# vsislab/Controllable_XGating

Measured on AMD Instinct MI355X. Metric: decoder timesteps/sec (train fwd+bwd) at batch 128, MSRVTT 26x1536+1024, higher is better.
Workload: dtype f32; 1 GPU; configs[1]: 1xMI355X batch 128 per GPU teacher-forced XE train, 26 frames x (1536+1024), hidden 512, att 1536, emb 468, vocab 20000, seq_len 20 (T=21), fp32; global_batch=128, per_gpu_batch=128, parallelism=dp1, gemm_precision=fp32, zero_grad=fused into the update, launch=eager kernel launches

## Files before the change

controllable_xgating_amd/csrc/xg_heads.hip:

```cpp
#include "xg_common.h"
#include "xg_kernels.h"
#include "xg_select.h"
#include <type_traits>
#include <cstdlib>

namespace {

constexpr int RT = 1024;

__device__ __forceinline__ float block_max(float v, float* red) {
    v = wave_max(v);
    const int lane = threadIdx.x & 63, wave = threadIdx.x >> 6;
    __syncthreads();
    if (lane == 0) red[wave] = v;
    __syncthreads();
    float r = red[0];
    for (int i = 1; i < (int)(blockDim.x >> 6); ++i) r = fmaxf(r, red[i]);
    return r;
}
__device__ __forceinline__ float block_sum(float v, float* red) {
    v = wave_sum(v);
    const int lane = threadIdx.x & 63, wave = threadIdx.x >> 6;
    __syncthreads();
    if (lane == 0) red[wave] = v;
// ... 110 lines not shown
    const float m = mask[i] * (mask2 ? mask2[i] : 1.f);
    dlogp[(size_t)i * V + tgt_of(target, b, t, T, roll)] = -scale * (scale_dev ? scale_dev[0] : 1.f) * m / sums[1];
}

__device__ __forceinline__ float reward_mask(const int64_t* seq, int ld_seq, int b, int t, int n) {
    if (t >= n) return 0.f;
    return (t == 0 || seq[(size_t)b * ld_seq + t - 1] > 0) ? 1.f : 0.f;
}
__global__ void reward_fwd_kernel(const float* slp, int ld_slp, const int64_t* seq, int ld_seq, const float* reward, int rs_b,
                                  int rs_t, const int32_t* n_dev, int m, int L, float* out2) {
    __shared__ float red[256 / 64];
    const int i = blockIdx.x * 256 + threadIdx.x;
    const int n = n_dev ? min(max(*n_dev, 0), L) : L;
    float a = 0.f, k = 0.f;
    if (i < m * L) {
        const int b = i / L, t = i % L;
        k = reward_mask(seq, ld_seq, b, t, n);
        if (k != 0.f) a = -slp[(size_t)b * ld_slp + t] * reward[(size_t)b * rs_b + (size_t)t * rs_t];
    }
    a = block_sum(a, red);
    k = block_sum(k, red);
    if (threadIdx.x == 0) { atomicAdd(out2, a); atomicAdd(out2 + 1, k); }
}
__global__ void reward_bwd_kernel(const int64_t* seq, int ld_seq, const float* reward, int rs_b, int rs_t, const int32_t* n_dev,
                                  int m, int L, const float* sums, const float* scale_dev, float* dslp, int ld_d) {
    const int i = blockIdx.x * 256 + threadIdx.x;
    if (i >= m * L) return;
    const int n = n_dev ? min(max(*n_dev, 0), L) : L;
    const int b = i / L, t = i % L;
    const float k = reward_mask(seq, ld_seq, b, t, n);
    dslp[(size_t)b * ld_d + t] = k != 0.f ? -(scale_dev ? scale_dev[0] : 1.f) * reward[(size_t)b * rs_b + (size_t)t * rs_t] / sums[1] : 0.f;
}

__device__ __forceinline__ void xent_row_finish(float mx, float s, float* red, const float* x, int i, int b, int t, int T,
                                                const int64_t* seq, const float* mask, const float* mask2, int roll,
                                                float* lse_out, float* sums2) {
    const float gmx = block_max(mx, red);
    s = (mx == -INFINITY) ? 0.f : s * expf(mx - gmx);
    s = block_sum(s, red);
    if (threadIdx.x == 0) {
        const float lse = gmx + logf(s);
        lse_out[i] = lse;
        const float m = mask[(size_t)b * T + t] * (mask2 ? mask2[(size_t)b * T + t] : 1.f);
        const int64_t tg = tgt_of(seq, b, t, T, roll);
        atomicAdd(sums2, -(x[tg] - lse) * m);
        atomicAdd(sums2 + 1, m);
    }
}
__global__ void __launch_bounds__(RT) xent_fwd_kernel(const float* __restrict__ logits, int ld, const int64_t* seq,
                                                        const float* mask, const float* mask2, int B, int T, int V,
                                                        int roll, float* lse_out, float* sums2, int row0) {
    __shared__ float red[RT / 64];
    const int i = row0 + blockIdx.x, t = i / B, b = i % B;
    const float* x = logits + (size_t)i * ld;
    float mx = -INFINITY, s = 0.f;
    for (int v0 = threadIdx.x; v0 < V; v0 += 8 * RT) {
        float xv[8];
#pragma unroll
        for (int j = 0; j < 8; ++j) { const int v = v0 + j * RT; xv[j] = v < V ? x[v] : -INFINITY; }
        float bm = xv[0];
#pragma unroll
        for (int j = 1; j < 8; ++j) bm = fmaxf(bm, xv[j]);
        if (bm > mx) { s *= expf(mx - bm); mx = bm; }
        if (mx > -INFINITY) {
#pragma unroll
            for (int j = 0; j < 8; ++j) s += expf(xv[j] - mx);
        }
    }
    xent_row_finish(mx, s, red, x, i, b, t, T, seq, mask, mask2, roll, lse_out, sums2);
}
template <int NV4>
__global__ void __launch_bounds__(RT) xent_fwd_reg_kernel(const float* __restrict__ logits, int ld, const int64_t* seq,
                                                            const float* mask, const float* mask2, int B, int T, int V,
                                                            int roll, float* lse_out, float* sums2, int row0) {
    __shared__ float red[RT / 64];
    const int i = row0 + blockIdx.x, t = i / B, b = i % B;
    const float* x = logits + (size_t)i * ld;
    float4 xv[NV4];
#pragma unroll
    for (int j = 0; j < NV4; ++j) {
        const int v = (threadIdx.x + j * RT) * 4;
        if (v + 3 < V) xv[j] = *reinterpret_cast<const float4*>(x + v);
        else {
            xv[j].x = v < V ? x[v] : -INFINITY;         xv[j].y = v + 1 < V ? x[v + 1] : -INFINITY;
            xv[j].z = v + 2 < V ? x[v + 2] : -INFINITY; xv[j].w = -INFINITY;
        }
    }
    float mx = -INFINITY;
#pragma unroll
    for (int j = 0; j < NV4; ++j) mx = fmaxf(fmaxf(mx, fmaxf(xv[j].x, xv[j].y)), fmaxf(xv[j].z, xv[j].w));
    float s = 0.f;
    if (mx > -INFINITY) {
#pragma unroll
        for (int j = 0; j < NV4; ++j) s += (expf(xv[j].x - mx) + expf(xv[j].y - mx)) + (expf(xv[j].z - mx) + expf(xv[j].w - mx));
    }
    xent_row_finish(mx, s, red, x, i, b, t, T, seq, mask, mask2, roll, lse_out, sums2);
}
template <bool BF>
__global__ void __launch_bounds__(RT) xent_bwd_kernel(float* __restrict__ logits, int ld, const int64_t* seq,
                                                        const float* mask, const float* mask2, int B, int T, int V,
                                                        int roll, const float* lse, const float* sums2,
                                                        const float* scale_dev, float scale, int row0, unsigned short* d16) {
    const int i = row0 + blockIdx.x, t = i / B, b = i % B;
    float* x = logits + (size_t)i * ld;
    const float m = mask[(size_t)b * T + t] * (mask2 ? mask2[(size_t)b * T + t] : 1.f);
    const float coef = (scale_dev ? scale_dev[0] : 1.f) * scale * m / sums2[1];
    const int64_t tg = tgt_of(seq, b, t, T, roll);
    const float l = lse[i];
    for (int v = threadIdx.x; v < V; v += RT) {
        const float pv = expf(x[v] - l);
        const float gv = coef * (pv - (v == tg ? 1.f : 0.f));
        x[v] = gv;
        if (BF) {
            unsigned u = __float_as_uint(gv);
            u += 0x7FFFu + ((u >> 16) & 1u);
            d16[(size_t)i * ld + v] = (unsigned short)(u >> 16);
        }
    }
}

template <int NV4, bool BF>
__global__ void __launch_bounds__(RT) xent_bwd_reg_kernel(float* __restrict__ logits, int ld, const int64_t* seq,
                                                            const float* mask, const float* mask2, int B, int T, int V,
                                                            int roll, const float* lse, const float* sums2,
                                                            const float* scale_dev, float scale, int row0, unsigned short* d16) {
    const int i = row0 + blockIdx.x, t = i / B, b = i % B;
    float* x = logits + (size_t)i * ld;
    float4 xv[NV4];
#pragma unroll
// ... 731 lines not shown
    else if (npt <= 16) hipLaunchKernelGGL((log_softmax_reg_kernel<16>), dim3(rows), dim3(RT), 0, st, in, ldin, out, ldout, V, inner, outer, pm);
    else if (npt <= 24) hipLaunchKernelGGL((log_softmax_reg_kernel<24>), dim3(rows), dim3(RT), 0, st, in, ldin, out, ldout, V, inner, outer, pm);
    else hipLaunchKernelGGL(log_softmax_kernel, dim3(rows), dim3(RT), 0, st, in, ldin, out, ldout, V, inner, outer, pm);
    XG_CHECK_LAUNCH();
    return XG_OK;
}
int xgk_log_softmax_bwd(hipStream_t st, const float* dlogp, const float* logp, int ldp, float* dlogits, int ldd,
                        int rows, int V, int inner, int outer, int permute) {
    if (rows <= 0) return XG_OK;
    const int npt = xg_cdiv(V, RT);
    if (npt <= 8) hipLaunchKernelGGL((log_softmax_bwd_reg_kernel<8>), dim3(rows), dim3(RT), 0, st, dlogp, logp, ldp, dlogits, ldd, V, inner, outer, permute);
    else if (npt <= 16) hipLaunchKernelGGL((log_softmax_bwd_reg_kernel<16>), dim3(rows), dim3(RT), 0, st, dlogp, logp, ldp, dlogits, ldd, V, inner, outer, permute);
    else if (npt <= 24) hipLaunchKernelGGL((log_softmax_bwd_reg_kernel<24>), dim3(rows), dim3(RT), 0, st, dlogp, logp, ldp, dlogits, ldd, V, inner, outer, permute);
    else hipLaunchKernelGGL(log_softmax_bwd_kernel, dim3(rows), dim3(RT), 0, st, dlogp, logp, ldp, dlogits, ldd, V, inner, outer, permute);
    XG_CHECK_LAUNCH();
    return XG_OK;
}
int xgk_nll_fwd(hipStream_t st, const float* logp, const int64_t* target, const float* mask, const float* mask2,
                int B, int T, int V, int roll, float* out2) {
    if (hipMemsetAsync(out2, 0, 2 * sizeof(float), st) != hipSuccess) return XG_EHIP;
    hipLaunchKernelGGL(nll_fwd_kernel, dim3(xg_cdiv(B * T, 256)), dim3(256), 0, st, logp, target, mask, mask2, B, T, V,
                       roll, out2);
    XG_CHECK_LAUNCH();
    return XG_OK;
}
int xgk_nll_bwd(hipStream_t st, const int64_t* target, const float* mask, const float* mask2, int B, int T, int V,
                int roll, const float* sums, float scale, const float* scale_dev, float* dlogp) {
    if (hipMemsetAsync(dlogp, 0, sizeof(float) * (size_t)B * T * V, st) != hipSuccess) return XG_EHIP;
    hipLaunchKernelGGL(nll_bwd_kernel, dim3(xg_cdiv(B * T, 256)), dim3(256), 0, st, target, mask, mask2, B, T, V, roll,
                       sums, scale, scale_dev, dlogp);
    XG_CHECK_LAUNCH();
    return XG_OK;
}
int xgk_xent_fwd(hipStream_t st, const float* logits, int ld, const int64_t* seq, const float* mask,
                 const float* mask2, int B, int T, int V, int roll, float* lse, float* sums2, int row0, int nrows,
                 bool zero_sums) {
    if (zero_sums && hipMemsetAsync(sums2, 0, 2 * sizeof(float), st) != hipSuccess) return XG_EHIP;
    if (nrows < 0) nrows = B * T - row0;
    if (nrows <= 0) return XG_OK;
    const bool al = ((uintptr_t)logits % 16 == 0) && ld % 4 == 0;
#define XG_XENT_REG(NV4_) hipLaunchKernelGGL((xent_fwd_reg_kernel<NV4_>), dim3(nrows), dim3(RT), 0, st, logits, ld, seq, mask, mask2, B, T, V, roll, lse, sums2, row0)
    if (al && V <= 2 * 4096) XG_XENT_REG(2);
    else if (al && V <= 5 * 4096) XG_XENT_REG(5);
    else if (al && V <= 8 * 4096) XG_XENT_REG(8);
    else hipLaunchKernelGGL(xent_fwd_kernel, dim3(nrows), dim3(RT), 0, st, logits, ld, seq, mask, mask2, B, T, V, roll, lse, sums2, row0);
#undef XG_XENT_REG
    XG_CHECK_LAUNCH();
    return XG_OK;
}
int xgk_xent_bwd(hipStream_t st, float* logits_inout, int ld, const int64_t* seq, const float* mask,
                 const float* mask2, int B, int T, int V, int roll, const float* lse, const float* sums2,
                 const float* scale_dev, float scale, int row0, int nrows, unsigned short* d16) {
    if (nrows < 0) nrows = B * T - row0;
    if (nrows <= 0) return XG_OK;
    const bool al = ((uintptr_t)logits_inout % 16 == 0) && ld % 4 == 0 && (!d16 || (uintptr_t)d16 % 8 == 0);
#define XG_XENT_BREG(NV4_) do { \
        if (d16) hipLaunchKernelGGL((xent_bwd_reg_kernel<NV4_, true>), dim3(nrows), dim3(RT), 0, st, logits_inout, ld, seq, mask, mask2, B, T, V, \
                                    roll, lse, sums2, scale_dev, scale, row0, d16); \
        else hipLaunchKernelGGL((xent_bwd_reg_kernel<NV4_, false>), dim3(nrows), dim3(RT), 0, st, logits_inout, ld, seq, mask, mask2, B, T, V, \
                                roll, lse, sums2, scale_dev, scale, row0, d16); } while (0)
    if (al && V > 1024 && V <= 2 * 4096) XG_XENT_BREG(2);
    else if (al && V > 1024 && V <= 5 * 4096) XG_XENT_BREG(5);
    else if (al && V > 1024 && V <= 8 * 4096) XG_XENT_BREG(8);
    else if (d16) hipLaunchKernelGGL(xent_bwd_kernel<true>, dim3(nrows), dim3(RT), 0, st, logits_inout, ld, seq, mask, mask2, B, T, V, roll,
                                     lse, sums2, scale_dev, scale, row0, d16);
    else hipLaunchKernelGGL(xent_bwd_kernel<false>, dim3(nrows), dim3(RT), 0, st, logits_inout, ld, seq, mask, mask2, B, T, V, roll,
                            lse, sums2, scale_dev, scale, row0, d16);
#undef XG_XENT_BREG
    XG_CHECK_LAUNCH();
    return XG_OK;
}
int xgk_choose(hipStream_t st, const float* logp, int B, int V, int mode, const float* uniforms,
               const int64_t* forced, int64_t forced_stride, float temperature, int64_t* tok, float* tok_logp) {
    hipLaunchKernelGGL(choose_kernel, dim3(B), dim3(RT), 0, st, logp, V, mode, uniforms, forced, forced_stride,
                       temperature, tok, tok_logp);
    XG_CHECK_LAUNCH();
    return XG_OK;
}
int xgk_rollout_step(hipStream_t st, int B, const float* logits, const float* uniforms, const int64_t* forced,
// ... 119 lines not shown
```

controllable_xgating_amd/csrc/xg_kernels.h:

```cpp
#pragma once
#include "xg_common.h"
#include "xg_select.h"
#include <cstddef>

static inline int xgk_group_rows(int k_depth) {
    const int g = 4096 / (k_depth > 0 ? k_depth : 1);
    return g < 1 ? 1 : (g > 8 ? 8 : g);
}
enum { XGK_GEMM_BG = 0x100,
       XGK_GEMM_ALONE = 0x200 };
int xgk_gemm(hipStream_t st, int mode, bool transA, bool transB, int M, int N, int K, const float* A, int lda,
             const float* B, int ldb, float* C, int ldc, const float* bias, bool relu, bool accumulate);
int xgk_gemm_cs(hipStream_t st, int mode, bool transA, bool transB, int M, int N, int K, const float* A, int lda,
                const float* B, int ldb, float* C, int ldc, const float* bias, bool relu, bool accumulate, float* cs1, float* cs2,
                float* cs3);
int xgk_gemm_x(hipStream_t st, int mode, bool transA, bool transB, int M, int N, int K, const float* A, const unsigned short* A16,
               int lda, const float* B, const unsigned short* B16, int ldb, float* C, int ldc, const float* bias, bool relu,
               bool accumulate, float* cs1 = nullptr, float* cs2 = nullptr, float* cs3 = nullptr);
int xgk_gemm_bf16(hipStream_t st, int planes, bool transA, bool transB, int M, int N, int K, const float* A, int lda,
                  const float* B, int ldb, float* C, int ldc, const float* bias, bool relu, bool accumulate, float* cs1 = nullptr,
                  float* cs2 = nullptr, float* cs3 = nullptr);
int xgk_gemm_bf16x(hipStream_t st, int planes, bool transA, bool transB, int M, int N, int K, const float* A, const unsigned short* A16,
                   int lda, const float* B, const unsigned short* B16, int ldb, float* C, int ldc, const float* bias, bool relu,
                   bool accumulate, float* cs1 = nullptr, float* cs2 = nullptr, float* cs3 = nullptr);
// ... 164 lines not shown
int xgk_dstep_err_word();
bool xgk_dstep_ok(const XgDims& d);
int xgk_dstep(hipStream_t st, DStepArgs& a, int gemm_mode);

enum { PK_H2A1 = 0, PK_H2A2, PK_DGATE, PK_L1_I2H, PK_L1_A2H, PK_L1_H2H, PK_L2_I2H, PK_L2_A2H, PK_L2_H2H, PK_ENC_RGB, PK_ENC_OPFL,
       PKB_L2_A2H, PKB_L2_H2H, PKB_H2A2, PKB_L1_H2H, PKB_ENC_RGB, PKB_ENC_OPFL, PKB_L2_I2H, PKB_H2A1, PK_COUNT };
enum { W16_LOGIT = 0, W16_EMB_RGB, W16_EMB_OPFL, W16_WIH_RGB, W16_WIH_OPFL, W16_GATE_RGB, W16_GATE_OPFL, W16_FUSION, W16_V2A,
       W16_DGATE, W16_L1_I2H, W16_L1_A2H, W16_COUNT };
struct PackedView { const float* m[PK_COUNT]; int nck[PK_COUNT]; int dtype;
                    const unsigned short* w16[W16_COUNT]; };
size_t xgk_packed_floats(const XgDims& d);
size_t xgk_packed_total_bytes(const XgDims& d, int dtype);
bool xgk_packed_view(const XgDims& d, const void* packed, int dtype, PackedView* v);

int xgk_attn_fwd(hipStream_t st, const float* p, const float* vproj, const float* V, const float* w, float* alpha,
                 float* af, int B, int K, int R, int A, bool half_cu = false);
int xgk_attn_bwd(hipStream_t st, const float* daf, int lddaf, const float* p, const float* vproj, const float* V,
                 const float* w, const float* alpha, float* de, float* dp, int B, int K, int R, int A);
int xgk_attn_bwd_post(hipStream_t st, const float* P , const float* vproj, const float* w,
                      const float* DE , float* dvproj, float* dw, int T, int B, int K, int A);
int xgk_attn_post_dV(hipStream_t st, const float* P, const float* vproj, const float* w, const float* DE, float* dvproj, float* dw,
                     const float* ALPHA, const float* DAF, int lddaf, int64_t daf_tstride, float* dV, int T, int B, int K, int A, int R);
int xgk_attn_dV(hipStream_t st, const float* ALPHA , const float* DAF , int lddaf,
                int64_t daf_tstride, float* dV, int T, int B, int K, int R, bool accumulate);

int xgk_log_softmax(hipStream_t st, const float* in, int ldin, float* out, int ldout, int rows, int V, int inner,
                    int outer, bool permute);
int xgk_log_softmax_bwd(hipStream_t st, const float* dlogp, const float* logp, int ldp, float* dlogits, int ldd,
                        int rows, int V, int inner, int outer, int permute);
int xgk_nll_fwd(hipStream_t st, const float* logp, const int64_t* target, const float* mask, const float* mask2,
                int B, int T, int V, int roll, float* out2);
int xgk_nll_bwd(hipStream_t st, const int64_t* target, const float* mask, const float* mask2, int B, int T, int V,
                int roll, const float* sums, float scale, const float* scale_dev, float* dlogp);
int xgk_xent_fwd(hipStream_t st, const float* logits, int ld, const int64_t* seq, const float* mask,
                 const float* mask2, int B, int T, int V, int roll, float* lse, float* sums2, int row0 = 0,
                 int nrows = -1, bool zero_sums = true);
int xgk_xent_bwd(hipStream_t st, float* logits_inout, int ld, const int64_t* seq, const float* mask,
                 const float* mask2, int B, int T, int V, int roll, const float* lse, const float* sums2,
                 const float* scale_dev, float scale, int row0 = 0, int nrows = -1, unsigned short* d16 = nullptr);
int xgk_choose(hipStream_t st, const float* logp, int B, int V, int mode, const float* uniforms,
               const int64_t* forced, int64_t forced_stride, float temperature, int64_t* tok, float* tok_logp);
int xgk_rollout_step(hipStream_t st, int B, const float* logits, const float* uniforms, const int64_t* forced,
                     int64_t fstride, const float* unf_prev, const float* table, int64_t* tok, float* tok_logp, float* unf,
                     float* lse, int64_t* seq, float* seq_logp, int32_t* maxf, float* xt, float temperature, int V, int E,
                     int t, int T, int mode, int split);
int xgk_rollout_finalize(hipStream_t st, const int32_t* maxf, int32_t* n_steps, int Tm1, int nparts);
bool xgk_vocab_select_ok(int B, int R, int V, const float* H, int ldh, const float* W);
int xgk_vocab_tile_width(int V);
int xgk_vocab_part(hipStream_t st, int B, int R, int V, const float* H, int ldh, const float* W, const float* bias, float* logits,
                   int wr_rows, float* part, float temperature);
RollSelectArgs xgk_roll_select_args(const float* logits, const float* part, const float* uniforms, const int64_t* forced, int64_t fstride,
                                    const float* unf_prev, const float* table, int64_t* tok, float* tok_logp, float* unf, float* lse,
                                    int64_t* seq, float* seq_logp, int32_t* maxf, float* xt, float temperature, int V, int E, int t, int T,
                                    int mode, int split);
int xgk_roll_select(hipStream_t st, int B, const float* logits, const float* part, const float* uniforms, const int64_t* forced,
                    int64_t fstride, const float* unf_prev, const float* table, int64_t* tok, float* tok_logp, float* unf,
                    float* lse, int64_t* seq, float* seq_logp, int32_t* maxf, float* xt, float temperature, int V, int E,
                    int t, int T, int mode, int split);
int xgk_rollout_dlogits_lse(hipStream_t st, float* logits, const float* lse, const int64_t* tok, const float* dslp,
                            int64_t dstride, int B, int V, int steps);
constexpr int XG_COMPACT_MAX = 48;
struct CompactEntry { float* dst; const float* src; int64_t dst_block, src_pitch, total; };
struct CompactArgs { int n; int start[XG_COMPACT_MAX + 1]; CompactEntry e[XG_COMPACT_MAX]; };
int xgk_compact(hipStream_t st, CompactArgs& a);
int xgk_ss_select(hipStream_t st, const int64_t* seq, int T, int t, int B, const float* u_sel, float ss_prob,
                  const int64_t* sampled, int64_t* tok);
int xgk_rollout_book(hipStream_t st, int t, int B, int Tm1, int replay, const int64_t* tok, const float* tok_logp,
                     float* unfinished, int64_t* seq, float* seq_logp, int32_t* n_steps, int32_t* alive);
int xgk_rollout_dlogits(hipStream_t st, const float* logp, const int64_t* tok, const float* dslp, int64_t dstride,
// ... 5 lines not shown
```

controllable_xgating_amd/csrc/xg_model.hip:

```cpp
#include "xg_common.h"
#include <cstring>
#include <ctime>
#include "xg_kernels.h"

#include <new>
#include <cstdlib>
#include <functional>

namespace {

constexpr int XG_NEV = 64, XG_NRING = 56;
struct XgAux { uint32_t magic; int device; hipStream_t s = nullptr, s2 = nullptr; hipEvent_t ev[XG_NEV]; };
constexpr uint32_t XG_AUX_MAGIC = 0x58474158u;
XgAux* aux_of(const XgRun* run) {
    static const bool disabled = xg_diag_env("XG_NO_OVERLAP") != nullptr;
    if (disabled || !run || !run->aux) return nullptr;
    XgAux* a = static_cast<XgAux*>(run->aux);
    int dev = -1;
    if (a->magic != XG_AUX_MAGIC || hipGetDevice(&dev) != hipSuccess || dev != a->device) return nullptr;
    return a;
}

struct Streams {
    hipStream_t main, aux, aux2;
// ... 710 lines not shown
    XG_TRY(lin16(sx, w.gm, TB, 4 * R, R, w.POSG, m16(w, w.POSG), R, p.l1_a2h_w, w16(w, W16_L1_A2H), p.l1_a2h_b, w.PRE1, 4 * R, false, true));
    return XG_OK;
}

int decoder_fwd_xe(Streams& ss, const XgDims& d, const XgParams& p, const XgBatch& x, const XgRun& run, Ws& w,
                   int* logit_rows_done, bool early_loss = false) {
    hipStream_t st = ss.main;
    const int B = d.B, R = d.R, A = d.A, E = d.E, T = d.T;
    const size_t BR = (size_t)B * R;
    XG_TRY(init_and_vproj(ss, d, p, x.feat_mask, w));
    XG_TRY(zero_dsync(st, w));
    XG_TRY(ss.join());
    const int th = (ss.overlap() && T >= 4) ? T / 2 : 0;
    const bool fwd_bg = th > 0 && w.gm == 0;
    *logit_rows_done = 0;
    if (run.prof_event0 && hipEventRecord(static_cast<hipEvent_t>(run.prof_event0), st) != hipSuccess) return XG_EHIP;
    for (int t = 0; t < T; ++t) {
        StepIO s{};
        s.xt = w.Xe + (size_t)t * B * E; s.posg = w.POSG + t * BR; s.pre1 = w.PRE1 + (size_t)t * B * 4 * R;
        s.mask = x.seq_mask + t; s.ldm = T;
        s.h1 = w.H1 + t * BR; s.c1 = w.C1 + t * BR; s.h2 = w.H2 + t * BR; s.c2 = w.C2 + t * BR;
        s.h1o = w.H1 + (t + 1) * BR; s.c1o = w.C1 + (t + 1) * BR; s.h2o = w.H2 + (t + 1) * BR; s.c2o = w.C2 + (t + 1) * BR;
        s.P = w.P + (size_t)t * B * A; s.alpha = w.ALPHA + (size_t)t * B * d.K; s.af = w.AF + t * BR;
        s.g1 = w.G1 + (size_t)t * B * 4 * R; s.g2 = w.G2 + (size_t)t * B * 4 * R; s.t = t;
        s.half_attn = fwd_bg;
        XG_TRY(core_step(st, d, p, run, w, w.Venc, w.vproj, s));
        if (th > 0 && t == th - 1) {
            XG_TRY(ss.fork());
            XG_TRY(cvt16(ss.aux, w, w.H2 + BR, (size_t)th * B * R));
            XG_TRY(lin16(ss.aux, w.gm | (fwd_bg ? XGK_GEMM_BG : 0), th * B, d.V, R, w.H2 + BR, m16(w, w.H2 + BR), R, p.logit_w,
                         w16(w, W16_LOGIT), p.logit_b, w.LOGITS, d.V));
            *logit_rows_done = th * B;
            if (early_loss)
                XG_TRY(xgk_xent_fwd(ss.aux, w.LOGITS, d.V, x.seq, x.seq_mask, nullptr, B, T, d.V, 1, w.LSE, w.sums, 0, th * B, false));
        }
    }
    if (run.prof_event1 && hipEventRecord(static_cast<hipEvent_t>(run.prof_event1), st) != hipSuccess) return XG_EHIP;
    return XG_OK;
}

int heads_fwd_logits(Streams& ss, const XgDims& d, const XgParams& p, const XgRun& run, Ws& w, int rows, int rows_done) {
    hipStream_t st = ss.main;
    const int B = d.B, R = d.R;
    const float* Hout = w.H2 + (size_t)B * R;
    XG_TRY(cvt16(st, w, Hout + (size_t)rows_done * R, (size_t)(rows - rows_done) * R));
    XG_TRY(lin16(st, w.gm, rows - rows_done, d.V, R, Hout + (size_t)rows_done * R, m16(w, Hout + (size_t)rows_done * R), R, p.logit_w,
                 w16(w, W16_LOGIT), p.logit_b, w.LOGITS + (size_t)rows_done * d.V, d.V));
    XG_TRY(xgk_linear(st, w.gm, rows, d.H, R, Hout, R, p.cls0_w, p.cls0_b, w.HC, d.H, true));
    XG_TRY(xgk_gate_fwd(st, w.HC, d.H, nullptr, 0, 0, nullptr, 0, rows, d.H, xg_make_drop(&run, XG_SITE_CLS, 0), B, 1 << 30,
                        1, B));
    XG_TRY(xgk_linear(st, w.gm, rows, d.C, d.H, w.HC, d.H, p.cls3_w, p.cls3_b, w.CL, d.C));
    return ss.join();
}

int decoder_bwd_core(Streams& ss, const XgDims& d, const XgParams& p, const XgParams& g, const XgBatch& x,
                     const XgRun& run, Ws& w, const float* mask, int ldm, int mask_tstride, const int64_t* tok,
                     int tok_bstride, int tok_tstride) {
    hipStream_t st = ss.main;
    const int B = d.B, K = d.K, R = d.R, A = d.A, E = d.E, T = d.T, TB = T * B, N = B * K;
    (void)TB;
    const size_t BR = (size_t)B * R;
    const bool fuse = R % 4 == 0;
    int cur = 0;
    if (w.zeroed) {
        XG_TRY(ss.join2());
    } else {
        for (int j = 0; j < 4; ++j) ZERO(w.dst[0][j], BR);
        ZERO(w.DAF, (size_t)T * BR);
        XG_TRY(zero_tickets(st, w, SK_MAX_JOBS));
    }
    auto cell2_bwd = [&](int t, int c) {
        LstmBwdArgs a{};
        a.gates = w.G2 + (size_t)t * B * 4 * R; a.ldg = 4 * R;
        a.c_prev = w.C2 + t * BR; a.ldcp = R; a.c_out = w.C2 + (t + 1) * BR; a.ldco = R;
        a.mask = mask + (size_t)t * mask_tstride; a.ldm = ldm;
        a.dh_out = w.dst[c][2]; a.lddh = R; a.dh_add = w.DH2OUT + t * BR; a.lddha = R;
        a.dc_out = w.dst[c][3]; a.lddc = R;
        a.ds = w.DS2 + (size_t)t * B * 4 * R; a.ldds = 4 * R;
        a.dc_prev = w.dst[c ^ 1][3]; a.lddcp = R; a.dh_prev = w.dst[c ^ 1][2]; a.lddhp = R;
        a.B = B; a.R = R; a.order = XG_ORDER_IFOG; a.mask_mode = XG_MASK_HOLD;
        a.drop = xg_make_drop(&run, XG_SITE_L2, t);
        return a;
    };
    hipStream_t s1 = ss.aux2;
// ... 145 lines not shown
        }
    }
    XG_TRY(wgrads_chain2(sx, 0, wg_hi));
    XG_TRY(wgrads_chain1(s1, 0, wg_hi));
    XG_TRY(ss.wait_mark2(wg_mark));
    XG_TRY(xgk_gate_bwd(s1, w.DPOSG, R, w.GP, R, x.pos_feats, R, B, w.DGP, R, nullptr, 0, false, TB, R,
                        xg_make_drop(&run, XG_SITE_DGATE, 0)));
    XG_TRY(gemm_tn_cs(s1, w.gm, TB, R, E, w.DGP, R, w.Xe, E, g.dgate_w, E, g.dgate_b));
    XG_TRY(gemm_nn(s1, w.gm, TB, E, R, w.DGP, R, p.dgate_w, E, w.DXe, E, true));
    XG_TRY(xgk_embed_scatter_add(s1, g.embed_w, E, tok, B, tok_bstride, tok_tstride, TB, d.V, w.DXe, E));
    XG_TRY(ss.fork());
    if (w.gm == 1) {
        XG_TRY(tn16(sx, w.gm, N, A, R, w.DVPROJ, m16(w, w.DVPROJ), A, w.Venc, m16(w, w.Venc), R, g.v2a_w, R));
        XG_TRY(xgk_colsum3(sx, w.DVPROJ, A, N, A, g.v2a_b, nullptr, nullptr));
    } else {
        XG_TRY(tn16(sx, w.gm, N, A, R, w.DVPROJ, m16(w, w.DVPROJ), A, w.Venc, m16(w, w.Venc), R, g.v2a_w, R, g.v2a_b));
    }
    XG_TRY(ss.chain2_into_aux());
    if (ss.grad_event && hipEventRecord(ss.grad_event, sx) != hipSuccess) return XG_EHIP;
    return XG_OK;
    };
    return tail();
}

int zero_backward_block(Streams& ss, Ws& w) {
    w.zeroed = false;
    if (!ss.overlap()) return XG_OK;
    XG_TRY(ss.fork2());
    if (hipMemsetAsync(w.zblock, 0, w.zbytes, ss.aux2) != hipSuccess) return XG_EHIP;
    w.zeroed = true;
    return XG_OK;
}

struct XentBwd { const int64_t* seq; const float* mask; const float* dloss_dev; };
int heads_bwd(Streams& ss, const XgDims& d, const XgParams& p, const XgParams& g, const XgRun& run, Ws& w, int rows,
              bool have_cls, const XentBwd* xent = nullptr) {
    hipStream_t st = ss.main;
    const int B = d.B, R = d.R, TB = d.T * B;
    const float* Hout = w.H2 + (size_t)B * R;
    XG_TRY(zero_backward_block(ss, w));
    if (rows < TB) ZERO(w.DH2OUT + (size_t)rows * R, (size_t)(TB - rows) * R);
    const int th = (ss.overlap() && !have_cls && rows == TB && d.T >= 4) ? d.T / 2 : 0;
    const int r0 = th * B;
    ss.dh_split_step = th; ss.dh_mark = -1;
    unsigned short* dl16 = const_cast<unsigned short*>(m16(w, w.LOGITS));
    if (xent) XG_TRY(xgk_xent_bwd(st, w.LOGITS, d.V, xent->seq, xent->mask, nullptr, B, d.T, d.V, 1, w.LSE, w.sums,
                                  xent->dloss_dev, 1.0f, r0, rows - r0, dl16));
    else XG_TRY(cvt16(st, w, w.LOGITS, (size_t)rows * d.V));
    XG_TRY(ss.fork());
    if (xent && r0 > 0) XG_TRY(xgk_xent_bwd(ss.aux, w.LOGITS, d.V, xent->seq, xent->mask, nullptr, B, d.T, d.V, 1, w.LSE,
                                            w.sums, xent->dloss_dev, 1.0f, 0, r0, dl16));
    XG_TRY(cvt16(st, w, Hout, (size_t)rows * R));
    const unsigned short* hout16 = m16(w, Hout);
    XG_TRY(nn16(st, w.gm, rows - r0, R, d.V, w.LOGITS + (size_t)r0 * d.V, m16(w, w.LOGITS + (size_t)r0 * d.V), d.V, p.logit_w,
                w16(w, W16_LOGIT), R, w.DH2OUT + (size_t)r0 * R, R, false));
    const int bgm = w.gm | (ss.overlap() && d.K <= 48 ? XGK_GEMM_BG : 0);
    XG_TRY(ss.fork());
    if (th > 0) {
        XG_TRY(nn16(ss.aux, bgm, r0, R, d.V, w.LOGITS, m16(w, w.LOGITS), d.V, p.logit_w, w16(w, W16_LOGIT), R, w.DH2OUT, R, false));
        ss.dh_mark = ss.mark();
        if (ss.dh_mark == -2) return XG_EHIP;
    }
    auto dwl = [=, &ss, &w, &g]() -> int {
        XG_TRY(tn16(ss.aux, bgm, rows, d.V, R, w.LOGITS, m16(w, w.LOGITS), d.V, Hout, hout16, R, g.logit_w, R, g.logit_b));
        if (ss.grad_event_head) {
            XG_TRY(ss.fork());
            if (hipEventRecord(ss.grad_event_head, ss.aux) != hipSuccess) return XG_EHIP;
        }
        return XG_OK;
    };
    XG_TRY(dwl());
    if (have_cls) {
        XG_TRY(gemm_tn_cs(st, w.gm, rows, d.C, d.H, w.DCL, d.C, w.HC, d.H, g.cls3_w, d.H, g.cls3_b));
        XG_TRY(gemm_nn(st, w.gm, rows, d.H, d.C, w.DCL, d.C, p.cls3_w, d.H, w.DHC, d.H, false));
        XG_TRY(xgk_relu_drop_bwd(st, w.DHC, w.HC, (int64_t)rows * d.H, xg_make_drop(&run, XG_SITE_CLS, 0)));
        XG_TRY(gemm_tn_cs(st, w.gm, rows, d.H, R, w.DHC, d.H, Hout, R, g.cls0_w, R, g.cls0_b));
        XG_TRY(gemm_nn(st, w.gm, rows, R, d.H, w.DHC, d.H, p.cls0_w, R, w.DH2OUT, R, true));
    }
    return XG_OK;
}

__global__ void losses_kernel(const float* s, float wc, float* out) {
    const float lx = s[0] / s[1];
    const float lc = s[3] > 0.f ? s[2] / s[3] : 0.f;
// ... 264 lines not shown
    c1.ds = w.DS1; c1.ldds = 4 * R; c1.dc_prev = dc1; c1.lddcp = R; c1.dh_prev = dh1; c1.lddhp = R;
    c1.B = B; c1.R = R; c1.order = XG_ORDER_IFOG; c1.mask_mode = XG_MASK_HOLD; c1.drop = xg_make_drop(run, XG_SITE_L1, step);
    XG_TRY(xgk_lstm_bwd(st, c1));
    XG_TRY(gemm_nn(st, 0, B, R, 4 * R, w.DS1, 4 * R, p->l1_h2h_w, R, dh1, R, true));
    XG_TRY(gemm_nn(st, 0, B, R, A, w.DP, A, p->h2a_w, 2 * R, dh1, R, true));
    XG_TRY(gemm_tn(st, 0, B, 4 * R, R, w.DS1, 4 * R, h1o, R, g->l1_h2h_w, R));
    XG_TRY(gemm_tn(st, 0, B, 4 * R, E, w.DS1, 4 * R, w.Xe, E, g->l1_i2h_w, E));
    XG_TRY(gemm_tn(st, 0, B, 4 * R, R, w.DS1, 4 * R, w.POSG, R, g->l1_a2h_w, R));
    XG_TRY(xgk_colsum3(st, w.DS1, 4 * R, B, 4 * R, g->l1_i2h_b, g->l1_a2h_b, g->l1_h2h_b));
    XG_TRY(gemm_nn(st, 0, B, R, 4 * R, w.DS1, 4 * R, p->l1_a2h_w, R, w.DPOSG, R, false));
    XG_TRY(gemm_nn(st, 0, B, E, 4 * R, w.DS1, 4 * R, p->l1_i2h_w, E, w.DXe, E, false));
    XG_TRY(xgk_gate_bwd(st, w.DPOSG, R, w.GP, R, pos_feats, R, 0, w.DGP, R, dpos, R, true, B, R, xg_make_drop(run, XG_SITE_DGATE, step)));
    XG_TRY(gemm_tn(st, 0, B, R, E, w.DGP, R, w.Xe, E, g->dgate_w, E));
    XG_TRY(xgk_colsum(st, w.DGP, R, B, R, g->dgate_b));
    XG_TRY(gemm_nn(st, 0, B, E, R, w.DGP, R, p->dgate_w, E, w.DXe, E, true));
    XG_TRY(xgk_embed_scatter_add(st, g->embed_w, E, tokens, B, 1, 0, B, d->V, w.DXe, E));
    return XG_OK;
}

extern "C" int xg_forward_xe(void* stream, const XgDims* d, const XgParams* p, const XgBnState* bn, const XgBatch* x,
                             const XgRun* run, void* ws, size_t ws_bytes, float* logp, float* cat_logp) {
    Ws w; XG_TRY(check(d, ws, ws_bytes, &w));
    if (!p || !x || !run || !logp || !x->seq || !x->seq_mask || !x->pos_feats) return XG_EINVAL;
    w.gm = (run->gemm_mode == 1 || run->gemm_mode == 3) ? run->gemm_mode : 0;
    attach_packed(w, *d, run);
    hipStream_t st = (hipStream_t)stream;
    const int TB = d->T * d->B;
    Streams ss(st, run);
    int rows_done = 0;
    XG_TRY(ss.fork());
    XG_TRY(decoder_tokens_xe(ss.aux, *d, *p, *x, *run, w));
    XG_TRY(encoder_fwd(st, *d, *p, bn, *x, *run, w, &ss));
    XG_TRY(decoder_fwd_xe(ss, *d, *p, *x, *run, w, &rows_done));
    XG_TRY(heads_fwd_logits(ss, *d, *p, *run, w, TB, rows_done));
    XG_TRY(xgk_log_softmax(st, w.LOGITS, d->V, logp, d->V, TB, d->V, d->B, d->T, true));
    if (cat_logp) XG_TRY(xgk_log_softmax(st, w.CL, d->C, cat_logp, d->C, TB, d->C, d->B, d->T, true));
    return XG_OK;
}

extern "C" int xg_backward_xe(void* stream, const XgDims* d, const XgParams* p, const XgParams* g, const XgBatch* x,
                              const XgRun* run, void* ws, size_t ws_bytes, const float* dlogp, const float* dcat_logp) {
    Ws w; XG_TRY(check(d, ws, ws_bytes, &w));
    if (!p || !g || !x || !run || !x->seq || !x->seq_mask) return XG_EINVAL;
    w.gm = (run->gemm_mode == 1 || run->gemm_mode == 3) ? run->gemm_mode : 0;
    attach_packed(w, *d, run);
    hipStream_t st = (hipStream_t)stream;
    const int B = d->B, T = d->T, TB = T * B;
    if (dlogp) {
        XG_TRY(xgk_log_softmax(st, w.LOGITS, d->V, w.LOGITS, d->V, TB, d->V, 1, 1, false));
        XG_TRY(xgk_log_softmax_bwd(st, dlogp, w.LOGITS, d->V, w.LOGITS, d->V, TB, d->V, B, T, 2));
    } else {
        ZERO(w.LOGITS, (size_t)TB * d->V);
    }
    if (dcat_logp) {
        XG_TRY(xgk_log_softmax(st, w.CL, d->C, w.CL, d->C, TB, d->C, 1, 1, false));
        XG_TRY(xgk_log_softmax_bwd(st, dcat_logp, w.CL, d->C, w.DCL, d->C, TB, d->C, B, T, 2));
    }
    Streams ss(st, run);
    XG_TRY(heads_bwd(ss, *d, *p, *g, *run, w, TB, dcat_logp != nullptr));
    XG_TRY(decoder_bwd_core(ss, *d, *p, *g, *x, *run, w, x->seq_mask, T, 1, x->seq, T, 1));
    XG_TRY(encoder_bwd(ss, *d, *p, *g, *x, *run, w, w.DV));
    return ss.join();
}

extern "C" int xg_forward_ss(void* stream, const XgDims* d, const XgParams* p, const XgBnState* bn, const XgBatch* x,
                             const XgRun* run, float ss_prob, const float* u_sel, const float* u_tok, void* ws,
                             size_t ws_bytes, float* logp, float* cat_logp) {
// ... 46 lines not shown
    Ws w; XG_TRY(check(d, ws, ws_bytes, &w));
    if (!p || !g || !x || !run || !x->seq || !x->seq_mask) return XG_EINVAL;
    w.gm = (run->gemm_mode == 1 || run->gemm_mode == 3) ? run->gemm_mode : 0;
    attach_packed(w, *d, run);
    hipStream_t st = (hipStream_t)stream;
    const int B = d->B, T = d->T, TB = T * B;
    if (dlogp) {
        XG_TRY(xgk_log_softmax_bwd(st, dlogp, w.LOGITS, d->V, w.LOGITS, d->V, TB, d->V, B, T, 2));
    } else {
        ZERO(w.LOGITS, (size_t)TB * d->V);
    }
    if (dcat_logp) {
        XG_TRY(xgk_log_softmax(st, w.CL, d->C, w.CL, d->C, TB, d->C, 1, 1, false));
        XG_TRY(xgk_log_softmax_bwd(st, dcat_logp, w.CL, d->C, w.DCL, d->C, TB, d->C, B, T, 2));
    }
    Streams ss(st, run);
    XG_TRY(heads_bwd(ss, *d, *p, *g, *run, w, TB, dcat_logp != nullptr));
    XG_TRY(decoder_bwd_core(ss, *d, *p, *g, *x, *run, w, x->seq_mask, T, 1, w.TOK, 1, B));
    XG_TRY(encoder_bwd(ss, *d, *p, *g, *x, *run, w, w.DV));
    return ss.join();
}

extern "C" int xg_xe_loss_fwd(void* stream, const XgDims* d, const XgParams* p, const XgBnState* bn, const XgBatch* x,
                              const int64_t* cap_classes, const float* class_mask, float weight_class, const XgRun* run,
                              void* ws, size_t ws_bytes, float* losses) {
    Ws w; XG_TRY(check(d, ws, ws_bytes, &w));
    if (!p || !x || !run || !losses || !x->seq || !x->seq_mask || !x->pos_feats) return XG_EINVAL;
    w.gm = (run->gemm_mode == 1 || run->gemm_mode == 3) ? run->gemm_mode : 0;
    attach_packed(w, *d, run);
    hipStream_t st = (hipStream_t)stream;
    const int TB = d->T * d->B;
    Streams ss(st, run);
    int rows_done = 0;
    ZERO(w.sums, 2);
    XG_TRY(ss.fork());
    XG_TRY(decoder_tokens_xe(ss.aux, *d, *p, *x, *run, w));
    XG_TRY(encoder_fwd(st, *d, *p, bn, *x, *run, w, &ss));
    XG_TRY(decoder_fwd_xe(ss, *d, *p, *x, *run, w, &rows_done, true));
    XG_TRY(heads_fwd_logits(ss, *d, *p, *run, w, TB, rows_done));
    XG_TRY(xgk_xent_fwd(st, w.LOGITS, d->V, x->seq, x->seq_mask, nullptr, d->B, d->T, d->V, 1, w.LSE, w.sums, rows_done, -1, false));
    if (cap_classes) {
        XG_TRY(xgk_xent_fwd(st, w.CL, d->C, cap_classes, x->seq_mask, class_mask, d->B, d->T, d->C, 0, w.LSEC, w.sums + 2));
    } else {
        ZERO(w.sums + 2, 2);
    }
    hipLaunchKernelGGL(losses_kernel, dim3(1), dim3(1), 0, st, w.sums, cap_classes ? weight_class : 0.f, losses);
    XG_CHECK_LAUNCH();
    return XG_OK;
}
extern "C" int xg_xe_loss_bwd(void* stream, const XgDims* d, const XgParams* p, const XgParams* g, const XgBatch* x,
                              const int64_t* cap_classes, const float* class_mask, float weight_class,
                              const float* dloss_dev, const XgRun* run, void* ws, size_t ws_bytes) {
    Ws w; XG_TRY(check(d, ws, ws_bytes, &w));
    if (!p || !g || !x || !run || !x->seq || !x->seq_mask) return XG_EINVAL;
    w.gm = (run->gemm_mode == 1 || run->gemm_mode == 3) ? run->gemm_mode : 0;
    attach_packed(w, *d, run);
    hipStream_t st = (hipStream_t)stream;
    const int B = d->B, T = d->T, TB = T * B;
    const XentBwd xent{x->seq, x->seq_mask, dloss_dev};
    const bool cls = cap_classes != nullptr && weight_class != 0.f;
    if (cls) {
        if (hipMemcpyAsync(w.DCL, w.CL, sizeof(float) * (size_t)TB * d->C, hipMemcpyDeviceToDevice, st) != hipSuccess) return XG_EHIP;
        XG_TRY(xgk_xent_bwd(st, w.DCL, d->C, cap_classes, x->seq_mask, class_mask, B, T, d->C, 0, w.LSEC, w.sums + 2,
                            dloss_dev, weight_class));
    }
    Streams ss(st, run);
    XG_TRY(heads_bwd(ss, *d, *p, *g, *run, w, TB, cls, &xent));
    XG_TRY(decoder_bwd_core(ss, *d, *p, *g, *x, *run, w, x->seq_mask, T, 1, x->seq, T, 1));
    XG_TRY(encoder_bwd(ss, *d, *p, *g, *x, *run, w, w.DV));
    return ss.join();
}

static int rollout_impl(hipStream_t st, const XgDims* d, const XgParams* p, const XgBnState* bn, const XgBatch* x,
                        const XgRun* run, int mode, const float* uniforms, const int64_t* forced, float temperature, Ws& w,
                        int64_t* seq, float* seq_logp, int32_t* n_steps, int split, float* logits_alt = nullptr,
                        bool* used_alt = nullptr, const XgDims* d1 = nullptr, Ws* enc = nullptr) {
    const int B = d->B, R = d->R, E = d->E, A = d->A, T = d->T;
    const size_t BR = (size_t)B * R;
    Streams es(st, run);
    const float* pos_rows = x->pos_feats;
    if (enc) {
        const size_t B1 = d1->B, N1 = B1 * d->K;
        XG_TRY(encoder_fwd(st, *d1, *p, bn, *x, *run, *enc, &es));
        if (run->train && bn && bn->rgb_mean && bn->rgb_var && bn->opfl_mean && bn->opfl_var) {
            XG_TRY(xgk_bn_running(st, enc->bn_mean[0], enc->bn_var[0], bn->rgb_mean, bn->rgb_var, (int)N1, R, run->bn_momentum));
            XG_TRY(xgk_bn_running(st, enc->bn_mean[1], enc->bn_var[1], bn->opfl_mean, bn->opfl_var, (int)N1, R, run->bn_momentum));
        }
        XG_TRY(init_and_vproj(es, *d1, *p, x->feat_mask, *enc));
        CompactArgs ca{};
        auto twice = [&](float* dst, const float* src, size_t n) {
            ca.e[ca.n++] = CompactEntry{dst, src, (int64_t)n, (int64_t)n, (int64_t)n};
            ca.e[ca.n++] = CompactEntry{dst + n, src, (int64_t)n, (int64_t)n, (int64_t)n};
// ... 208 lines not shown
```

Baseline: 504,200 decoder timesteps/s.

## Fuse cross-entropy gradient into forward pass and precompute mask sum

The forward cross-entropy kernel now writes the softmax gradient (and its bf16 copy) straight into the logits buffer when saving for backward. It can do this because the mask normalizer is computed up front by a small init kernel. Backward then only rescales by the loss gradient, and skips even that when the scale is 1. This removes a second full read of the logits and the exp recomputation in backward. The class head is also skipped when no caption classes are given. In exchange, the forward pass does extra writes, the backward path changes structure, and it now depends on the presummed mask being correct.

```diff
diff --git a/controllable_xgating_amd/csrc/xg_heads.hip b/controllable_xgating_amd/csrc/xg_heads.hip
--- a/controllable_xgating_amd/csrc/xg_heads.hip
+++ b/controllable_xgating_amd/csrc/xg_heads.hip
@@ -166,27 +166,42 @@
     dslp[(size_t)b * ld_d + t] = k != 0.f ? -(scale_dev ? scale_dev[0] : 1.f) * reward[(size_t)b * rs_b + (size_t)t * rs_t] / sums[1] : 0.f;
 }
 
-__device__ __forceinline__ void xent_row_finish(float mx, float s, float* red, const float* x, int i, int b, int t, int T,
-                                                const int64_t* seq, const float* mask, const float* mask2, int roll,
-                                                float* lse_out, float* sums2) {
+__global__ void __launch_bounds__(256) xent_sums_init_kernel(const float* __restrict__ mask, int n, float* sums2) {
+    __shared__ float red[256 / 64];
+    float a = 0.f;
+    for (int i = threadIdx.x; i < n; i += 256) a += mask[i];
+    a = block_sum(a, red);
+    if (threadIdx.x == 0) { sums2[0] = 0.f; sums2[1] = a; sums2[2] = 0.f; sums2[3] = 0.f; }
+}
+__device__ __forceinline__ unsigned short xent_bf16(float gv) {
+    unsigned u = __float_as_uint(gv);
+    u += 0x7FFFu + ((u >> 16) & 1u);
+    return (unsigned short)(u >> 16);
+}
+__device__ __forceinline__ float xent_row_finish(float mx, float s, float* red, float xtg, int i, float m, bool presummed,
+                                                 float* lse_out, float* sums2) {
     const float gmx = block_max(mx, red);
     s = (mx == -INFINITY) ? 0.f : s * expf(mx - gmx);
     s = block_sum(s, red);
+    const float lse = gmx + logf(s);
     if (threadIdx.x == 0) {
-        const float lse = gmx + logf(s);
         lse_out[i] = lse;
-        const float m = mask[(size_t)b * T + t] * (mask2 ? mask2[(size_t)b * T + t] : 1.f);
-        const int64_t tg = tgt_of(seq, b, t, T, roll);
-        atomicAdd(sums2, -(x[tg] - lse) * m);
-        atomicAdd(sums2 + 1, m);
-    }
-}
-__global__ void __launch_bounds__(RT) xent_fwd_kernel(const float* __restrict__ logits, int ld, const int64_t* seq,
+        atomicAdd(sums2, -(xtg - lse) * m);
+        if (!presummed) atomicAdd(sums2 + 1, m);
+    }
+    return lse;
+}
+template <int G>
+__global__ void __launch_bounds__(RT) xent_fwd_kernel(float* __restrict__ logits, int ld, const int64_t* seq,
                                                         const float* mask, const float* mask2, int B, int T, int V,
-                                                        int roll, float* lse_out, float* sums2, int row0) {
+                                                        int roll, float* lse_out, float* sums2, int row0, bool presummed,
+                                                        unsigned short* d16) {
     __shared__ float red[RT / 64];
     const int i = row0 + blockIdx.x, t = i / B, b = i % B;
-    const float* x = logits + (size_t)i * ld;
+    float* x = logits + (size_t)i * ld;
+    const float m = mask[(size_t)b * T + t] * (mask2 ? mask2[(size_t)b * T + t] : 1.f);
+    const int64_t tg = tgt_of(seq, b, t, T, roll);
+    const float xtg = threadIdx.x == 0 ? x[tg] : 0.f;
     float mx = -INFINITY, s = 0.f;
     for (int v0 = threadIdx.x; v0 < V; v0 += 8 * RT) {
         float xv[8];
@@ -201,15 +216,33 @@
             for (int j = 0; j < 8; ++j) s += expf(xv[j] - mx);
         }
     }
-    xent_row_finish(mx, s, red, x, i, b, t, T, seq, mask, mask2, roll, lse_out, sums2);
-}
-template <int NV4>
-__global__ void __launch_bounds__(RT) xent_fwd_reg_kernel(const float* __restrict__ logits, int ld, const int64_t* seq,
+    const float l = xent_row_finish(mx, s, red, xtg, i, m, presummed, lse_out, sums2);
+    if (G) {
+        const float coef = m / sums2[1];
+        for (int v0 = threadIdx.x; v0 < V; v0 += 8 * RT) {
+            float xv[8];
+#pragma unroll
+            for (int j = 0; j < 8; ++j) { const int v = v0 + j * RT; xv[j] = v < V ? x[v] : 0.f; }
+#pragma unroll
+            for (int j = 0; j < 8; ++j) {
+                const int v = v0 + j * RT;
+                if (v < V) {
+                    const float gv = coef * (expf(xv[j] - l) - (v == tg ? 1.f : 0.f));
+                    x[v] = gv;
+                    if (G == 2) d16[(size_t)i * ld + v] = xent_bf16(gv);
+                }
+            }
+        }
+    }
+}
+template <int NV4, int G>
+__global__ void __launch_bounds__(RT) xent_fwd_reg_kernel(float* __restrict__ logits, int ld, const int64_t* seq,
                                                             const float* mask, const float* mask2, int B, int T, int V,
-                                                            int roll, float* lse_out, float* sums2, int row0) {
+                                                            int roll, float* lse_out, float* sums2, int row0, bool presummed,
+                                                            unsigned short* d16) {
     __shared__ float red[RT / 64];
     const int i = row0 + blockIdx.x, t = i / B, b = i % B;
-    const float* x = logits + (size_t)i * ld;
+    float* x = logits + (size_t)i * ld;
     float4 xv[NV4];
 #pragma unroll
     for (int j = 0; j < NV4; ++j) {
@@ -220,6 +253,9 @@
             xv[j].z = v + 2 < V ? x[v + 2] : -INFINITY; xv[j].w = -INFINITY;
         }
     }
+    const float m = mask[(size_t)b * T + t] * (mask2 ? mask2[(size_t)b * T + t] : 1.f);
+    const int tg = (int)tgt_of(seq, b, t, T, roll);
+    const float xtg = threadIdx.x == 0 ? x[tg] : 0.f;
     float mx = -INFINITY;
 #pragma unroll
     for (int j = 0; j < NV4; ++j) mx = fmaxf(fmaxf(mx, fmaxf(xv[j].x, xv[j].y)), fmaxf(xv[j].z, xv[j].w));
@@ -228,7 +264,52 @@
 #pragma unroll
         for (int j = 0; j < NV4; ++j) s += (expf(xv[j].x - mx) + expf(xv[j].y - mx)) + (expf(xv[j].z - mx) + expf(xv[j].w - mx));
     }
-    xent_row_finish(mx, s, red, x, i, b, t, T, seq, mask, mask2, roll, lse_out, sums2);
+    const float l = xent_row_finish(mx, s, red, xtg, i, m, presummed, lse_out, sums2);
+    if (G) {
+        const float coef = m / sums2[1];
+#pragma unroll
+        for (int j = 0; j < NV4; ++j) {
+            const int v = (threadIdx.x + j * RT) * 4;
+            float4 gq;
+            gq.x = coef * (expf(xv[j].x - l) - (v == tg ? 1.f : 0.f));
+            gq.y = coef * (expf(xv[j].y - l) - (v + 1 == tg ? 1.f : 0.f));
+            gq.z = coef * (expf(xv[j].z - l) - (v + 2 == tg ? 1.f : 0.f));
+            gq.w = coef * (expf(xv[j].w - l) - (v + 3 == tg ? 1.f : 0.f));
+            if (v + 3 < V) {
+                *reinterpret_cast<float4*>(x + v) = gq;
+                if (G == 2) {
+                    ushort4 h; h.x = xent_bf16(gq.x); h.y = xent_bf16(gq.y); h.z = xent_bf16(gq.z); h.w = xent_bf16(gq.w);
+                    *reinterpret_cast<ushort4*>(d16 + (size_t)i * ld + v) = h;
+                }
+            } else {
+                const float ga[3] = {gq.x, gq.y, gq.z};
+                for (int q = 0; q < 3 && v + q < V; ++q) {
+                    x[v + q] = ga[q];
+                    if (G == 2) d16[(size_t)i * ld + v + q] = xent_bf16(ga[q]);
+                }
+            }
+        }
+    }
+}
+__global__ void __launch_bounds__(256) xent_scale_kernel(float* __restrict__ x, unsigned short* __restrict__ d16, size_t n,
+                                                          size_t n4, const float* scale_dev) {
+    const float sc = scale_dev[0];
+    if (sc == 1.0f) return;
+    const size_t stride = (size_t)gridDim.x * 256, i0 = (size_t)blockIdx.x * 256 + threadIdx.x;
+    for (size_t q = i0; q < n4; q += stride) {
+        float4 g = reinterpret_cast<float4*>(x)[q];
+        g.x *= sc; g.y *= sc; g.z *= sc; g.w *= sc;
+        reinterpret_cast<float4*>(x)[q] = g;
+        if (d16) {
+            ushort4 h; h.x = xent_bf16(g.x); h.y = xent_bf16(g.y); h.z = xent_bf16(g.z); h.w = xent_bf16(g.w);
+            reinterpret_cast<ushort4*>(d16)[q] = h;
+        }
+    }
+    for (size_t e = n4 * 4 + i0; e < n; e += stride) {
+        const float g = x[e] * sc;
+        x[e] = g;
+        if (d16) d16[e] = xent_bf16(g);
+    }
 }
 template <bool BF>
 __global__ void __launch_bounds__(RT) xent_bwd_kernel(float* __restrict__ logits, int ld, const int64_t* seq,
@@ -1026,19 +1107,38 @@
     XG_CHECK_LAUNCH();
     return XG_OK;
 }
-int xgk_xent_fwd(hipStream_t st, const float* logits, int ld, const int64_t* seq, const float* mask,
+int xgk_xent_sums_init(hipStream_t st, const float* mask, int n, float* sums2) {
+    hipLaunchKernelGGL(xent_sums_init_kernel, dim3(1), dim3(256), 0, st, mask, n, sums2);
+    XG_CHECK_LAUNCH();
+    return XG_OK;
+}
+int xgk_xent_fwd(hipStream_t st, float* logits, int ld, const int64_t* seq, const float* mask,
                  const float* mask2, int B, int T, int V, int roll, float* lse, float* sums2, int row0, int nrows,
-                 bool zero_sums) {
+                 bool zero_sums, bool presummed, bool write_grad, unsigned short* d16) {
+    if (write_grad && !presummed) return XG_EINVAL;
     if (zero_sums && hipMemsetAsync(sums2, 0, 2 * sizeof(float), st) != hipSuccess) return XG_EHIP;
     if (nrows < 0) nrows = B * T - row0;
     if (nrows <= 0) return XG_OK;
-    const bool al = ((uintptr_t)logits % 16 == 0) && ld % 4 == 0;
-#define XG_XENT_REG(NV4_) hipLaunchKernelGGL((xent_fwd_reg_kernel<NV4_>), dim3(nrows), dim3(RT), 0, st, logits, ld, seq, mask, mask2, B, T, V, roll, lse, sums2, row0)
+    const int G = !write_grad ? 0 : d16 ? 2 : 1;
+    const bool al = ((uintptr_t)logits % 16 == 0) && ld % 4 == 0 && (G != 2 || (uintptr_t)d16 % 8 == 0);
+#define XG_XENT_L(...) hipLaunchKernelGGL((__VA_ARGS__), dim3(nrows), dim3(RT), 0, st, logits, ld, seq, mask, mask2, B, T, V, roll, lse, sums2, row0, presummed, d16)
+#define XG_XENT_G(K_) do { if (G == 0) XG_XENT_L(K_<0>); else if (G == 1) XG_XENT_L(K_<1>); else XG_XENT_L(K_<2>); } while (0)
+#define XG_XENT_REG(NV4_) do { if (G == 0) XG_XENT_L(xent_fwd_reg_kernel<NV4_, 0>); else if (G == 1) XG_XENT_L(xent_fwd_reg_kernel<NV4_, 1>); \
+        else XG_XENT_L(xent_fwd_reg_kernel<NV4_, 2>); } while (0)
     if (al && V <= 2 * 4096) XG_XENT_REG(2);
     else if (al && V <= 5 * 4096) XG_XENT_REG(5);
-    else if (al && V <= 8 * 4096) XG_XENT_REG(8);
-    else hipLaunchKernelGGL(xent_fwd_kernel, dim3(nrows), dim3(RT), 0, st, logits, ld, seq, mask, mask2, B, T, V, roll, lse, sums2, row0);
+    else if (al && V <= 8 * 4096 && G == 0) XG_XENT_L(xent_fwd_reg_kernel<8, 0>);
+    else XG_XENT_G(xent_fwd_kernel);
 #undef XG_XENT_REG
+#undef XG_XENT_G
+#undef XG_XENT_L
+    XG_CHECK_LAUNCH();
+    return XG_OK;
+}
+int xgk_xent_scale(hipStream_t st, float* x, unsigned short* d16, size_t n, const float* scale_dev) {
+    if (n == 0 || !scale_dev) return XG_OK;
+    const bool al = ((uintptr_t)x % 16 == 0) && (!d16 || (uintptr_t)d16 % 8 == 0);
+    hipLaunchKernelGGL(xent_scale_kernel, dim3(512), dim3(256), 0, st, x, d16, n, al ? n / 4 : (size_t)0, scale_dev);
     XG_CHECK_LAUNCH();
     return XG_OK;
 }
diff --git a/controllable_xgating_amd/csrc/xg_kernels.h b/controllable_xgating_amd/csrc/xg_kernels.h
--- a/controllable_xgating_amd/csrc/xg_kernels.h
+++ b/controllable_xgating_amd/csrc/xg_kernels.h
@@ -220,9 +220,12 @@
                 int B, int T, int V, int roll, float* out2);
 int xgk_nll_bwd(hipStream_t st, const int64_t* target, const float* mask, const float* mask2, int B, int T, int V,
                 int roll, const float* sums, float scale, const float* scale_dev, float* dlogp);
-int xgk_xent_fwd(hipStream_t st, const float* logits, int ld, const int64_t* seq, const float* mask,
+int xgk_xent_sums_init(hipStream_t st, const float* mask, int n, float* sums2);
+int xgk_xent_fwd(hipStream_t st, float* logits, int ld, const int64_t* seq, const float* mask,
                  const float* mask2, int B, int T, int V, int roll, float* lse, float* sums2, int row0 = 0,
-                 int nrows = -1, bool zero_sums = true);
+                 int nrows = -1, bool zero_sums = true, bool presummed = false, bool write_grad = false,
+                 unsigned short* d16 = nullptr);
+int xgk_xent_scale(hipStream_t st, float* x, unsigned short* d16, size_t n, const float* scale_dev);
 int xgk_xent_bwd(hipStream_t st, float* logits_inout, int ld, const int64_t* seq, const float* mask,
                  const float* mask2, int B, int T, int V, int roll, const float* lse, const float* sums2,
                  const float* scale_dev, float scale, int row0 = 0, int nrows = -1, unsigned short* d16 = nullptr);
diff --git a/controllable_xgating_amd/csrc/xg_model.hip b/controllable_xgating_amd/csrc/xg_model.hip
--- a/controllable_xgating_amd/csrc/xg_model.hip
+++ b/controllable_xgating_amd/csrc/xg_model.hip
@@ -766,24 +766,27 @@
                          w16(w, W16_LOGIT), p.logit_b, w.LOGITS, d.V));
             *logit_rows_done = th * B;
             if (early_loss)
-                XG_TRY(xgk_xent_fwd(ss.aux, w.LOGITS, d.V, x.seq, x.seq_mask, nullptr, B, T, d.V, 1, w.LSE, w.sums, 0, th * B, false));
+                XG_TRY(xgk_xent_fwd(ss.aux, w.LOGITS, d.V, x.seq, x.seq_mask, nullptr, B, T, d.V, 1, w.LSE, w.sums, 0, th * B, false,
+                                    true, run.save != 0, run.save ? const_cast<unsigned short*>(m16(w, w.LOGITS)) : nullptr));
         }
     }
     if (run.prof_event1 && hipEventRecord(static_cast<hipEvent_t>(run.prof_event1), st) != hipSuccess) return XG_EHIP;
     return XG_OK;
 }
 
-int heads_fwd_logits(Streams& ss, const XgDims& d, const XgParams& p, const XgRun& run, Ws& w, int rows, int rows_done) {
+int heads_fwd_logits(Streams& ss, const XgDims& d, const XgParams& p, const XgRun& run, Ws& w, int rows, int rows_done, bool cls) {
     hipStream_t st = ss.main;
     const int B = d.B, R = d.R;
     const float* Hout = w.H2 + (size_t)B * R;
     XG_TRY(cvt16(st, w, Hout + (size_t)rows_done * R, (size_t)(rows - rows_done) * R));
     XG_TRY(lin16(st, w.gm, rows - rows_done, d.V, R, Hout + (size_t)rows_done * R, m16(w, Hout + (size_t)rows_done * R), R, p.logit_w,
                  w16(w, W16_LOGIT), p.logit_b, w.LOGITS + (size_t)rows_done * d.V, d.V));
-    XG_TRY(xgk_linear(st, w.gm, rows, d.H, R, Hout, R, p.cls0_w, p.cls0_b, w.HC, d.H, true));
-    XG_TRY(xgk_gate_fwd(st, w.HC, d.H, nullptr, 0, 0, nullptr, 0, rows, d.H, xg_make_drop(&run, XG_SITE_CLS, 0), B, 1 << 30,
-                        1, B));
-    XG_TRY(xgk_linear(st, w.gm, rows, d.C, d.H, w.HC, d.H, p.cls3_w, p.cls3_b, w.CL, d.C));
+    if (cls) {
+        XG_TRY(xgk_linear(st, w.gm, rows, d.H, R, Hout, R, p.cls0_w, p.cls0_b, w.HC, d.H, true));
+        XG_TRY(xgk_gate_fwd(st, w.HC, d.H, nullptr, 0, 0, nullptr, 0, rows, d.H, xg_make_drop(&run, XG_SITE_CLS, 0), B, 1 << 30,
+                            1, B));
+        XG_TRY(xgk_linear(st, w.gm, rows, d.C, d.H, w.HC, d.H, p.cls3_w, p.cls3_b, w.CL, d.C));
+    }
     return ss.join();
 }
 
@@ -995,7 +998,7 @@
     return XG_OK;
 }
 
-struct XentBwd { const int64_t* seq; const float* mask; const float* dloss_dev; };
+struct XentBwd { const float* dloss_dev; };
 int heads_bwd(Streams& ss, const XgDims& d, const XgParams& p, const XgParams& g, const XgRun& run, Ws& w, int rows,
               bool have_cls, const XentBwd* xent = nullptr) {
     hipStream_t st = ss.main;
@@ -1007,12 +1010,11 @@
     const int r0 = th * B;
     ss.dh_split_step = th; ss.dh_mark = -1;
     unsigned short* dl16 = const_cast<unsigned short*>(m16(w, w.LOGITS));
-    if (xent) XG_TRY(xgk_xent_bwd(st, w.LOGITS, d.V, xent->seq, xent->mask, nullptr, B, d.T, d.V, 1, w.LSE, w.sums,
-                                  xent->dloss_dev, 1.0f, r0, rows - r0, dl16));
+    if (xent) XG_TRY(xgk_xent_scale(st, w.LOGITS + (size_t)r0 * d.V, dl16 ? dl16 + (size_t)r0 * d.V : nullptr,
+                                    (size_t)(rows - r0) * d.V, xent->dloss_dev));
     else XG_TRY(cvt16(st, w, w.LOGITS, (size_t)rows * d.V));
     XG_TRY(ss.fork());
-    if (xent && r0 > 0) XG_TRY(xgk_xent_bwd(ss.aux, w.LOGITS, d.V, xent->seq, xent->mask, nullptr, B, d.T, d.V, 1, w.LSE,
-                                            w.sums, xent->dloss_dev, 1.0f, 0, r0, dl16));
+    if (xent && r0 > 0) XG_TRY(xgk_xent_scale(ss.aux, w.LOGITS, dl16, (size_t)r0 * d.V, xent->dloss_dev));
     XG_TRY(cvt16(st, w, Hout, (size_t)rows * R));
     const unsigned short* hout16 = m16(w, Hout);
     XG_TRY(nn16(st, w.gm, rows - r0, R, d.V, w.LOGITS + (size_t)r0 * d.V, m16(w, w.LOGITS + (size_t)r0 * d.V), d.V, p.logit_w,
@@ -1343,7 +1345,7 @@
     XG_TRY(decoder_tokens_xe(ss.aux, *d, *p, *x, *run, w));
     XG_TRY(encoder_fwd(st, *d, *p, bn, *x, *run, w, &ss));
     XG_TRY(decoder_fwd_xe(ss, *d, *p, *x, *run, w, &rows_done));
-    XG_TRY(heads_fwd_logits(ss, *d, *p, *run, w, TB, rows_done));
+    XG_TRY(heads_fwd_logits(ss, *d, *p, *run, w, TB, rows_done, true));
     XG_TRY(xgk_log_softmax(st, w.LOGITS, d->V, logp, d->V, TB, d->V, d->B, d->T, true));
     if (cat_logp) XG_TRY(xgk_log_softmax(st, w.CL, d->C, cat_logp, d->C, TB, d->C, d->B, d->T, true));
     return XG_OK;
@@ -1456,18 +1458,16 @@
     const int TB = d->T * d->B;
     Streams ss(st, run);
     int rows_done = 0;
-    ZERO(w.sums, 2);
+    XG_TRY(xgk_xent_sums_init(st, x->seq_mask, TB, w.sums));
     XG_TRY(ss.fork());
     XG_TRY(decoder_tokens_xe(ss.aux, *d, *p, *x, *run, w));
     XG_TRY(encoder_fwd(st, *d, *p, bn, *x, *run, w, &ss));
     XG_TRY(decoder_fwd_xe(ss, *d, *p, *x, *run, w, &rows_done, true));
-    XG_TRY(heads_fwd_logits(ss, *d, *p, *run, w, TB, rows_done));
-    XG_TRY(xgk_xent_fwd(st, w.LOGITS, d->V, x->seq, x->seq_mask, nullptr, d->B, d->T, d->V, 1, w.LSE, w.sums, rows_done, -1, false));
-    if (cap_classes) {
+    XG_TRY(heads_fwd_logits(ss, *d, *p, *run, w, TB, rows_done, cap_classes != nullptr));
+    XG_TRY(xgk_xent_fwd(st, w.LOGITS, d->V, x->seq, x->seq_mask, nullptr, d->B, d->T, d->V, 1, w.LSE, w.sums, rows_done, -1, false,
+                        true, run->save != 0, run->save ? const_cast<unsigned short*>(m16(w, w.LOGITS)) : nullptr));
+    if (cap_classes)
         XG_TRY(xgk_xent_fwd(st, w.CL, d->C, cap_classes, x->seq_mask, class_mask, d->B, d->T, d->C, 0, w.LSEC, w.sums + 2));
-    } else {
-        ZERO(w.sums + 2, 2);
-    }
     hipLaunchKernelGGL(losses_kernel, dim3(1), dim3(1), 0, st, w.sums, cap_classes ? weight_class : 0.f, losses);
     XG_CHECK_LAUNCH();
     return XG_OK;
@@ -1481,7 +1481,7 @@
     attach_packed(w, *d, run);
     hipStream_t st = (hipStream_t)stream;
     const int B = d->B, T = d->T, TB = T * B;
-    const XentBwd xent{x->seq, x->seq_mask, dloss_dev};
+    const XentBwd xent{dloss_dev};
     const bool cls = cap_classes != nullptr && weight_class != 0.f;
     if (cls) {
         if (hipMemcpyAsync(w.DCL, w.CL, sizeof(float) * (size_t)TB * d->C, hipMemcpyDeviceToDevice, st) != hipSuccess) return XG_EHIP;
```

Measured after the change: 495,000 decoder timesteps/s. -1.8%, worse.
